# RLinf/RLinf

Measured on NVIDIA H100. Metric: env-steps/sec (rollout+update), higher is better.
Workload: dtype f32

## Files before the change

rlinf_b200/csrc/mlp.cu:

```cuda
#include <curand_kernel.h>

#include "common.cuh"
#include "sgemm.cuh"
#include "tc_gemm.cuh"

namespace {

using namespace rb::gemm;

__global__ void __launch_bounds__(256) colsum_kernel(const float* __restrict__ Z, float* __restrict__ out, int64_t M, int N,
                                                     int64_t rows_per_block) {
  const int64_t r0 = (int64_t)blockIdx.x * rows_per_block;
  const int64_t r1 = (r0 + rows_per_block < M) ? r0 + rows_per_block : M;
  for (int n = threadIdx.x; n < N; n += blockDim.x) {
    float s0 = 0.f, s1 = 0.f, s2 = 0.f, s3 = 0.f;
    int64_t r = r0;
    for (; r + 3 < r1; r += 4) {
      s0 += Z[r * N + n];
      s1 += Z[(r + 1) * N + n];
      s2 += Z[(r + 2) * N + n];
      s3 += Z[(r + 3) * N + n];
    }
    for (; r < r1; ++r) s0 += Z[r * N + n];
    atomicAdd(&out[n], (s0 + s1) + (s2 + s3));
// ... 309 lines not shown
    }
    if (lane == 0) {
      if (mz > 0.f) atomicMax(reinterpret_cast<unsigned int*>(p.amax_dz3), __float_as_uint(mz));
      if (has_v && my > 0.f && p.amax_dy3) atomicMax(reinterpret_cast<unsigned int*>(p.amax_dy3), __float_as_uint(my));
    }
  }
#pragma unroll
  for (int j = 0; j < 4; ++j) {
    atomicAdd(&a_b2[lane * 4 + j], cb[j]);
    atomicAdd(&a_b2[128 + lane * 4 + j], cb[4 + j]);
    if (has_v) {
      atomicAdd(&a_vb2[lane * 4 + j], cv[j]);
      atomicAdd(&a_vb2[128 + lane * 4 + j], cv[4 + j]);
    }
  }
  if (REG) {
#pragma unroll
    for (int a = 0; a < 8; ++a) {
      if (a >= p.act) break;
      float* am = a_mw + a * kH;
#pragma unroll
      for (int j = 0; j < 4; ++j) {
        atomicAdd(&am[lane * 4 + j], rm[a][j]);
        atomicAdd(&am[128 + lane * 4 + j], rm[a][4 + j]);
      }
    }
    if (has_v) {
#pragma unroll
      for (int c = 0; c < 2; ++c) {
        if (c >= p.vdim) break;
        float* av = a_vw + c * kH;
#pragma unroll
        for (int j = 0; j < 4; ++j) {
          atomicAdd(&av[lane * 4 + j], rv[c][j]);
          atomicAdd(&av[128 + lane * 4 + j], rv[c][4 + j]);
        }
      }
    }
  }
  __syncthreads();
  for (int i = threadIdx.x; i < acc_len; i += blockDim.x) {
    float s = 0.f;
    for (int w = 0; w < nwarp; ++w) s += acc0[w * acc_len + i];
    p.part[(size_t)blockIdx.x * acc_len + i] = s;
  }
}

int head_grid(int64_t n) {
  int64_t blocks = (n + 7) / 8;
  const int64_t cap = (int64_t)rb::sm_count() * 4;
  if (blocks > cap) blocks = cap;
  return (int)(blocks < 1 ? 1 : blocks);
}

struct TowerW {
  const float *w0, *b0, *w1, *b1, *w2, *b2;
};
int layer_forward(const float* in, const int64_t* idx, int64_t n, int in_dim, const float* w, const float* b,
                  float* out, cudaStream_t st) {
  GemmArgs g{};
  g.M = n; g.N = kH; g.ldc = kH; g.k_per_split = 1 << 30;
  g.A = in; g.lda = in_dim; g.a_rows = idx; g.B = w; g.ldb = in_dim; g.K = in_dim; g.bias = b; g.C = out;
  return launch_gemm<A_KCONTIG, B_KCONTIG, EPI_BIAS_TANH>(g, 1, st);
}

int tower_forward(const float* X, const int64_t* idx, int64_t n, int in_dim, const TowerW& w, float* H1, float* H2,
                  float* H3, cudaStream_t st) {
  int e = layer_forward(X, idx, n, in_dim, w.w0, w.b0, H1, st);
  if (e) return e;
  e = layer_forward(H1, nullptr, n, kH, w.w1, w.b1, H2, st);
  if (e) return e;
  return layer_forward(H2, nullptr, n, kH, w.w2, w.b2, H3, st);
}

int tower_backward(const float* X, const int64_t* idx, int64_t n, int in_dim, const TowerW& w, const float* H1, const float* H2, const float* dZ3, float* tmpA, float* tmpB, float* g_w0,
                   float* g_b0, float* g_w1, float* g_b1, float* g_w2, float* g_b2, cudaStream_t st) {
  const int64_t rows_per_split = 4096;
  const int splits = (int)((n + rows_per_split - 1) / rows_per_split);
  const int64_t cs_rows = 128;
  const int cs_blocks = (int)((n + cs_rows - 1) / cs_rows);
  int e;
  auto colsum = [&](const float* dZ, float* gb) -> int {
    colsum_kernel<<<cs_blocks, 256, 0, st>>>(dZ, gb, n, kH, cs_rows);
    rb::count_launch();
    cudaError_t ce = cudaPeekAtLastError();
    return ce == cudaSuccess ? 0 : (int)ce;
  };
  auto wgrad = [&](const float* dZ, const float* Hin, const int64_t* in_rows, int in_ld, float* gw, float* gb,
                   bool need_colsum) -> int {
    GemmArgs g{};
    g.A = dZ; g.lda = kH; g.B = Hin; g.ldb = in_ld; g.b_rows = in_rows; g.C = gw;
    g.ldc = in_ld; g.M = kH; g.N = in_ld; g.K = n; g.k_per_split = rows_per_split;
    const int ee = launch_gemm<A_MCONTIG, B_NCONTIG, EPI_ATOMIC>(g, splits, st);
    if (ee || !need_colsum) return ee;
    return colsum(dZ, gb);
  };
  auto dgrad = [&](const float* dZ, const float* W, const float* Hprev, float* out) -> int {
    GemmArgs g{};
    g.A = dZ; g.lda = kH; g.B = W; g.ldb = kH; g.C = out; g.ldc = kH; g.aux = Hprev;
    g.ldaux = kH; g.M = n; g.N = kH; g.K = kH; g.k_per_split = 1 << 30;
    return launch_gemm<A_KCONTIG, B_NCONTIG, EPI_TANHGRAD>(g, 1, st);
  };
  if ((e = wgrad(dZ3, H2, nullptr, kH, g_w2, g_b2, false))) return e;
  if ((e = dgrad(dZ3, w.w2, H2, tmpA))) return e;
  if ((e = wgrad(tmpA, H1, nullptr, kH, g_w1, g_b1, true))) return e;
  if ((e = dgrad(tmpA, w.w1, H1, tmpB))) return e;
  return wgrad(tmpB, X, idx, in_dim, g_w0, g_b0, true);
}


struct TowerWH {
  const float *w0f, *w1f, *w2f;
  const float *w1d, *w2d;
};

struct TowerIO {
  TowerW w;
  TowerWH wh;
  float *H1, *H2, *H3;
  float *g_w0, *g_b0, *g_w1, *g_b1, *g_w2, *g_b2;
  const float* dZ3;
  float *tA, *tB;
  float* amax;
};

bool layer0_on_tc(const int64_t* idx, int in_dim) { return idx == nullptr && in_dim % rb::tc::BK == 0; }

float* x_amax_slot(const rb200_mlp_layout* L, float* buf, int64_t n) { return buf + 6 * n * kH + n * L->act_dim; }
int64_t x_amax_floats(int cols) { return cols <= 256 ? 4 + cols : 1; }

int publish_absmax(const float* X, int64_t rows, int cols, float* out, cudaStream_t st) {
  if (reinterpret_cast<uintptr_t>(X) & 15) return RB200_E_ALIGN;
  if (cols % 4 != 0) return RB200_E_SHAPE;
  cudaError_t ce = cudaMemsetAsync(out, 0, sizeof(float) * x_amax_floats(cols), st);
  if (ce != cudaSuccess) return (int)ce;
  const int cols4 = cols / 4, col_out = cols <= 256 ? cols : 0;
  const int threads = col_out ? cols4 * (256 / cols4) : 256;
  const int64_t n4 = rows * cols4;
  int64_t blocks = (n4 + threads - 1) / threads;
  const int64_t cap = (int64_t)rb::sm_count() * 4;
  if (blocks > cap) blocks = cap;
  absmax_kernel<<<(int)(blocks < 1 ? 1 : blocks), threads, 0, st>>>(reinterpret_cast<const float4*>(X), n4,
                                                                    col_out ? cols4 : 1, col_out, out);
  rb::count_launch();
  ce = cudaPeekAtLastError();
  return ce == cudaSuccess ? 0 : (int)ce;
}

int towers_forward_h(const float* X, const int64_t* idx, int64_t n, int in_dim, TowerIO* t, int nt, float* x_amax,
                     const float* x_amax_in, cudaStream_t st) {
  int e;
  const bool l0_tc = layer0_on_tc(idx, in_dim);
  rb::tch::GemmLaunch g[2];
  if (l0_tc) {
    if (x_amax_in) {
      cudaError_t ce = cudaMemcpyAsync(x_amax, x_amax_in, sizeof(float) * x_amax_floats(in_dim), cudaMemcpyDeviceToDevice, st);
      if (ce != cudaSuccess) return (int)ce;
    } else if ((e = publish_absmax(X, n, in_dim, x_amax, st))) {
      return e;
    }
    for (int i = 0; i < nt; ++i) g[i] = rb::tch::GemmLaunch{X, t[i].wh.w0f, nullptr, t[i].H1, t[i].w.b0, nullptr, nullptr, nullptr, nullptr, x_amax};
    if ((e = rb::tch::launch(g, nt, n, in_dim, rb::tc::EPI_BIAS_TANH, 0, st))) return e;
  } else {
    for (int i = 0; i < nt; ++i)
      if ((e = layer_forward(X, idx, n, in_dim, t[i].w.w0, t[i].w.b0, t[i].H1, st))) return e;
  }
  for (int i = 0; i < nt; ++i) g[i] = rb::tch::GemmLaunch{t[i].H1, t[i].wh.w1f, nullptr, t[i].H2, t[i].w.b1, nullptr, nullptr, nullptr, nullptr};
  if ((e = rb::tch::launch(g, nt, n, kH, rb::tc::EPI_BIAS_TANH, 0, st))) return e;
  for (int i = 0; i < nt; ++i) g[i] = rb::tch::GemmLaunch{t[i].H2, t[i].wh.w2f, nullptr, t[i].H3, t[i].w.b2, nullptr, nullptr, nullptr, nullptr};
  return rb::tch::launch(g, nt, n, kH, rb::tc::EPI_BIAS_TANH, 0, st);
}

int simt_wgrad_chunks(int64_t n, int64_t* rows_per_chunk) {
  int64_t chunks = (n + 255) / 256;
  const int64_t cap = rb::sm_count() / 2 > 1 ? rb::sm_count() / 2 : 1;
  if (chunks > cap) chunks = cap;
  const int64_t rows = (n + chunks - 1) / chunks;
  *rows_per_chunk = rows;
  return (int)((n + rows - 1) / rows);
}

int towers_backward_h(const float* X, const int64_t* idx, int64_t n, int in_dim, TowerIO* t, int nt,
                      const float* x_amax, cudaStream_t st) {
  int e;
  rb::tch::WgradLaunch w[2];
  rb::tch::BackwardLaunch b[2];
  for (int i = 0; i < nt; ++i)
    b[i] = rb::tch::BackwardLaunch{t[i].dZ3, t[i].wh.w2d, t[i].H2, t[i].tA, t[i].g_w2, t[i].g_b1, t[i].amax, t[i].amax + 1,
                                   t[i].tB};
  if ((e = rb::tch::dgrad_wgrad(b, nt, n, st))) return e;
  for (int i = 0; i < nt; ++i)
    b[i] = rb::tch::BackwardLaunch{t[i].tA, t[i].wh.w1d, t[i].H1, t[i].tB, t[i].g_w1, t[i].g_b0, t[i].amax + 1, t[i].amax + 2,
                                   const_cast<float*>(t[i].dZ3)};
  if ((e = rb::tch::dgrad_wgrad(b, nt, n, st))) return e;
  if (layer0_on_tc(idx, in_dim) && in_dim <= 256) {
    for (int i = 0; i < nt; ++i) w[i] = rb::tch::WgradLaunch{t[i].tB, X, t[i].g_w0, t[i].amax + 2, x_amax + 4};
    return rb::tch::wgrad(w, nt, n, in_dim, st);
  }
  int64_t rows = 0;
  const int chunks = simt_wgrad_chunks(n, &rows);
  const int64_t slab = (int64_t)kH * in_dim;
  float* part = rb::partials_scratch(chunks * slab);
  if (!part) return RB200_E_UNSUPPORTED;
  for (int i = 0; i < nt; ++i) {
    GemmArgs a{};
    a.A = t[i].tB; a.lda = kH; a.B = X; a.ldb = in_dim; a.b_rows = idx; a.C = part; a.c_split_stride = slab;
    a.ldc = in_dim; a.M = kH; a.N = in_dim; a.K = n; a.k_per_split = rows;
    if ((e = launch_gemm<A_MCONTIG, B_NCONTIG, EPI_STORE>(a, chunks, st))) return e;
    rb::tch::SlotSums ss{};
    ss.count = 1;
    ss.nslab = chunks;
    ss.stride = slab;
    ss.part[0] = part;
    ss.out[0] = t[i].g_w0;
    ss.len[0] = (int)slab;
    if ((e = rb::tch::sum_slots(ss, st))) return e;
  }
  return 0;
}

}

extern "C" int rb200_mlp_layout_init(rb200_mlp_layout* L, int obs_dim, int act_dim, int value_dim, int hidden) {
  if (!L) return RB200_E_NULL;
  if (obs_dim <= 0 || act_dim <= 0 || value_dim < 0) return RB200_E_SHAPE;
  if (hidden != kH || act_dim > kMaxAct || value_dim > kMaxVal) return RB200_E_UNSUPPORTED;
  L->obs_dim = obs_dim; L->act_dim = act_dim; L->value_dim = value_dim; L->hidden = hidden;
  int64_t o = 0;
  auto take = [&](int64_t n) { o = (o + 3) & ~int64_t(3); const int64_t at = o; o += n; return at; };
  L->logstd = take(act_dim);
  L->vw0 = take((int64_t)hidden * obs_dim); L->vb0 = take(hidden);
  L->vw1 = take((int64_t)hidden * hidden); L->vb1 = take(hidden);
  L->vw2 = take((int64_t)hidden * hidden); L->vb2 = take(hidden);
  L->vw3 = take((int64_t)value_dim * hidden);
  L->bw0 = take((int64_t)hidden * obs_dim); L->bb0 = take(hidden);
  L->bw1 = take((int64_t)hidden * hidden); L->bb1 = take(hidden);
  L->bw2 = take((int64_t)hidden * hidden); L->bb2 = take(hidden);
  L->mw = take((int64_t)act_dim * hidden); L->mb = take(act_dim);
  L->total = (o + 3) & ~int64_t(3);
  const int64_t sms = rb::sm_count(), head = 4 * sms * ((act_dim + value_dim) * hidden + 64 + 2 * hidden);
  const int64_t wg = sms / 2 * hidden * (obs_dim > hidden ? obs_dim : hidden) + sms * hidden;
  if (!rb::partials_scratch(head > wg ? head : wg)) (void)cudaGetLastError();
  return RB200_OK;
}

static inline int64_t act_floats(int64_t n) { return n * kH; }

extern "C" int64_t rb200_mlp_fwd_scratch_floats(const rb200_mlp_layout* L, int64_t n) {
  if (!L || n <= 0) return 0;
  return 6 * act_floats(n) + n * L->act_dim + 64 + 256;
}

static inline int64_t wsplit_tower_floats(int obs) { return (int64_t)kH * obs + 4ll * kH * kH; }

extern "C" int64_t rb200_mlp_wsplit_floats(const rb200_mlp_layout* L) {
  if (!L) return 0;
  return 2 * wsplit_tower_floats(L->obs_dim);
}

static int check_layout(const rb200_mlp_layout* L) {
  if (!L) return RB200_E_NULL;
  if (L->hidden != kH || L->act_dim <= 0 || L->act_dim > kMaxAct || L->value_dim < 0 || L->value_dim > kMaxVal)
    return RB200_E_UNSUPPORTED;
  return RB200_OK;
}

namespace {
TowerW tower_w(const rb200_mlp_layout* L, const float* P, bool value) {
  TowerW w;
  if (value) {
    w.w0 = P + L->vw0; w.b0 = P + L->vb0; w.w1 = P + L->vw1; w.b1 = P + L->vb1; w.w2 = P + L->vw2; w.b2 = P + L->vb2;
  } else {
    w.w0 = P + L->bw0; w.b0 = P + L->bb0; w.w1 = P + L->bw1; w.b1 = P + L->bb1; w.w2 = P + L->bw2; w.b2 = P + L->bb2;
  }
  return w;
}
TowerWH tower_wh(const rb200_mlp_layout* L, const float* ws, bool value) {
  const int64_t n0 = (int64_t)kH * L->obs_dim, nn = (int64_t)kH * kH;
  const float* b = ws + (value ? 0 : wsplit_tower_floats(L->obs_dim));
  TowerWH t;
  t.w0f = b;
  t.w1f = b + n0;
  t.w2f = b + n0 + nn;
  t.w1d = b + n0 + 2 * nn;
  t.w2d = b + n0 + 3 * nn;
  return t;
}
}

extern "C" int rb200_mlp_prepare_weights(const rb200_mlp_layout* L, const float* params, float* wsplit,
                                         rb200_stream_t stream) {
  int e = check_layout(L);
  if (e) return e;
  if (!params || !wsplit) return RB200_E_NULL;
  rb::tch::SplitSpec sp[6];
  int cnt = 0;
  for (int v = 0; v < 2; ++v) {
    if (v == 0 && L->value_dim == 0) continue;
    const TowerW w = tower_w(L, params, v == 0);
    const TowerWH t = tower_wh(L, wsplit, v == 0);
    const int64_t n0 = (int64_t)kH * L->obs_dim, nn = (int64_t)kH * kH;
    if (L->obs_dim % rb::tc::BK == 0)
      sp[cnt++] = rb::tch::SplitSpec{w.w0, const_cast<float*>(t.w0f), nullptr, n0};
    sp[cnt++] = rb::tch::SplitSpec{w.w1, const_cast<float*>(t.w1f), const_cast<float*>(t.w1d), nn};
    sp[cnt++] = rb::tch::SplitSpec{w.w2, const_cast<float*>(t.w2f), const_cast<float*>(t.w2d), nn};
  }
  return rb::tch::split_weights(sp, cnt, rb::as_stream(stream));
}

extern "C" int rb200_mlp_forward(const rb200_mlp_layout* L, const float* params, const float* wsplit,
                                 const float* states, const float* action, const int64_t* idx, int64_t n,
                                 float* logprobs, float* entropy, float* values, float* acts, float* work,
                                 const float* states_amax, rb200_stream_t stream) {
  int e = check_layout(L);
  if (e) return e;
  if (!params || !states || !action || !logprobs || !acts || !work) return RB200_E_NULL;
  if (n <= 0) return RB200_E_SHAPE;
  if (values && L->value_dim == 0) return RB200_E_SHAPE;
  cudaStream_t st = rb::as_stream(stream);
  const int64_t PF = act_floats(n);
  float *H1 = acts, *H2 = H1 + PF, *H3 = H2 + PF, *G1 = H3 + PF, *G2 = G1 + PF, *G3 = G2 + PF;
  float* mean = G3 + PF;
  const float* P = params;
// ... 219 lines not shown
```

rlinf_b200/csrc/tc_gemm.cuh:

```cuda
#pragma once
#include <cuda_runtime.h>
#include <stdint.h>

namespace rb {
namespace tc {

constexpr int BM = 128, BN = 256, BK = 32;

enum Epi { EPI_STORE = 0, EPI_BIAS_TANH = 1, EPI_TANHGRAD = 2 };

extern int g_debug_flags;

}

namespace tch {

struct GemmLaunch {
  const float* a;
  const float* b_hi;
  const float* b_lo;
  float* c;
  const float* bias;
  const float* h;
  float* colsum;
  const float* amax_in;
  float* amax_out;
  const float* amax_x;
};
struct WgradLaunch {
  const float* z;
  const float* h;
  float* dW;
  const float* amax_z;
  const float* amax_h;
};
struct SplitSpec {
  const float* src;
  float* hi;
  float* lo;
  int64_t n;
};

int launch(const GemmLaunch* groups, int ngroups, int64_t M, int K, int epi, int b_mn, cudaStream_t st);
int wgrad(const WgradLaunch* groups, int ngroups, int64_t n, int IN, cudaStream_t st);
struct BackwardLaunch {
  const float* z;
  const float* wpack;
  const float* h;
  float* dzprev;
  float* dW;
  float* colsum;
  const float* amax_in;
  float* amax_out;
  float* scratch;
};
int dgrad_wgrad(const BackwardLaunch* groups, int ngroups, int64_t n, cudaStream_t st);
int split_weights(const SplitSpec* specs, int count, cudaStream_t st);
struct SlotSums {
  const float* part[8];
  float* out[8];
  int len[8];
  int count, nslab;
  int64_t stride;
};
int sum_slots(const SlotSums& s, cudaStream_t st);

}
}
```

rlinf_b200/csrc/tc_gemm_h.cu:

```cuda
#include <cuda_fp16.h>

#include "common.cuh"
#include "tc_gemm.cuh"
#include "tc_half.cuh"
#include "tma.cuh"
#include "wgmma.cuh"

namespace rb {
namespace tch {

using rb::tc::BK;
using rb::tc::BM;
using rb::tc::BN;

constexpr int kStages = 4;
constexpr int kA32 = BM * BK * 4;
constexpr int kB16 = BN * BK * 2;
constexpr int kWBytes = 2 * kB16;
constexpr int kStageBytes = kA32 + kWBytes;
constexpr int kRingBytes = kStages * kStageBytes;
constexpr int kThreads = 384;
constexpr int kProducerRegs = 40, kConsumerRegs = 232;
static_assert(128 * kProducerRegs + 256 * kConsumerRegs <= 65536, "register file");

__device__ __forceinline__ float tanh_fast(float x) {
  const float t = __expf(-2.0f * fabsf(x));
  return copysignf(__fdividef(1.0f - t, 1.0f + t), x);
}

__device__ __forceinline__ void a_frag_rows(const uint8_t* tile, int r0, int c0, float scale, uint32_t (&hi)[4],
                                            uint32_t (&lo)[4]) {
#pragma unroll
  for (int i = 0; i < 4; ++i) {
    const int r = r0 + (i & 1) * 8, c = c0 + (i >> 1) * 8;
    const float2 x = *reinterpret_cast<const float2*>(tile + r * 128 + ((((c >> 2) ^ (r & 7))) << 4) + (c & 3) * 4);
    split2(x.x * scale, x.y * scale, hi[i], lo[i]);
  }
}

struct __align__(16) Barriers {
  uint64_t full[kStages];
  uint64_t empty[kStages];
  alignas(16) float bias[BN];
  float csum[8][BN];
};

struct Group {
  const float* bias;
  const float* h;
  float* colsum;
  const float* amax_in;
  const float* amax_x;
  float* amax_out;
  float* c;
};

struct GemmParams {
  CUtensorMap a[2];
  const uint8_t* wpack[2];
  Group g[2];
  float* part;
  int64_t M;
  int K;
  int epi;
  int ngroups;
};

template <int B_MN>
__global__ void __launch_bounds__(kThreads, 1) tc_h_gemm_kernel(const __grid_constant__ GemmParams P) {
  extern __shared__ uint8_t smem_raw[];
  uint8_t* smem = smem_raw + ((1024u - (tma::smem_u32(smem_raw) & 1023u)) & 1023u);
  Barriers* bars = reinterpret_cast<Barriers*>(smem + kRingBytes);

  const int wg = threadIdx.x >> 7, warp = threadIdx.x >> 5, lane = threadIdx.x & 31;
  const int grp = blockIdx.x % P.ngroups;
  const int cta = blockIdx.x / P.ngroups, n_cta = gridDim.x / P.ngroups;
  const Group& G = P.g[grp];
  const int64_t n_tiles = (P.M + BM - 1) / BM;
  const int n_kb = P.K / BK;

  if (threadIdx.x == 0) {
    for (int s = 0; s < kStages; ++s) {
      tma::mbar_init(&bars->full[s], 1);
      tma::mbar_init(&bars->empty[s], 8);
    }
    tma::fence_barrier_init();
  }
  for (int i = threadIdx.x; i < BN; i += kThreads) bars->bias[i] = (P.epi == rb::tc::EPI_BIAS_TANH) ? G.bias[i] : 0.f;
  for (int i = threadIdx.x; i < 8 * BN; i += kThreads) bars->csum[i / BN][i % BN] = 0.f;
  __syncthreads();

  if (wg == 2) {
    wg::setmaxnreg_dec<kProducerRegs>();
    if (threadIdx.x == 256) {
      tma::prefetch_desc(&P.a[grp]);
      uint32_t s = 0, ph = 0;
      for (int64_t tile = cta; tile < n_tiles; tile += n_cta) {
        for (int kb = 0; kb < n_kb; ++kb) {
          tma::mbar_wait(&bars->empty[s], ph ^ 1u);
          uint8_t* st = smem + s * kStageBytes;
          tma::mbar_arrive_expect_tx(&bars->full[s], kStageBytes);
          tma::load_2d(st, &P.a[grp], kb * BK, (int)(tile * BM), &bars->full[s]);
          bulk_load(st + kA32, P.wpack[grp] + (size_t)kb * kWBytes, kWBytes, &bars->full[s]);
          if (++s == kStages) { s = 0; ph ^= 1u; }
        }
      }
    }
  } else {
    wg::setmaxnreg_inc<kConsumerRegs>();
    const int cw = wg;
    const int g = lane >> 2, t = lane & 3;
    const int r_lo = cw * 64 + (warp & 3) * 16 + g;
    const int sa = G.amax_in ? scale_log2_for(__ldg(G.amax_in)) : (G.amax_x ? input_scale_log2_for(__ldg(G.amax_x)) : 0);
    const float a_scale = pow2i(sa);
    const float out_scale = pow2i(-(sa + kWeightScaleLog2));
    float vmax = 0.f;
    auto load_a = [&](uint32_t q, uint32_t(&ah)[BK / 16][4], uint32_t(&al)[BK / 16][4]) {
      tma::mbar_wait_brk(&bars->full[q % kStages], (q / kStages) & 1u);
      const uint8_t* st = smem + (q % kStages) * kStageBytes;
#pragma unroll
      for (int k = 0; k < BK / 16; ++k) a_frag_rows(st, r_lo, k * 16 + 2 * t, a_scale, ah[k], al[k]);
    };
    uint32_t q0 = 0;
    for (int64_t tile = cta; tile < n_tiles; tile += n_cta) {
      float acc[128];
#pragma unroll
      for (int i = 0; i < 128; ++i) acc[i] = 0.f;
      auto step = [&](int kb, const uint32_t(&ah)[BK / 16][4], const uint32_t(&al)[BK / 16][4],
                      uint32_t(&nh)[BK / 16][4], uint32_t(&nl)[BK / 16][4]) {
        const uint32_t q = q0 + kb;
        const uint32_t wbase = tma::smem_u32(smem + (q % kStages) * kStageBytes + kA32);
        wg::fence();
#pragma unroll
        for (int k = 0; k < BK / 16; ++k) {
          const uint64_t b_hi = B_MN ? wg::desc(wbase + k * 2048, 4096, 1024, kSw128) : wg::desc(wbase + k * 32, 16, 512, kSw64);
          const uint64_t b_lo = B_MN ? wg::desc(wbase + kB16 + k * 2048, 4096, 1024, kSw128)
                                     : wg::desc(wbase + kB16 + k * 32, 16, 512, kSw64);
          wg::Mma<256, B_MN>::run(acc, al[k], b_hi, 1u);
          wg::Mma<256, B_MN>::run(acc, ah[k], b_lo, 1u);
          wg::Mma<256, B_MN>::run(acc, ah[k], b_hi, 1u);
        }
        wg::commit();
        wg::wait<1>();
        if (kb > 0) warp_arrive(&bars->empty[(q - 1) % kStages]);
        if (kb + 1 < n_kb) load_a(q + 1, nh, nl);
      };
      uint32_t ah0[BK / 16][4], al0[BK / 16][4], ah1[BK / 16][4], al1[BK / 16][4];
      load_a(q0, ah0, al0);
      for (int kb = 0; kb < n_kb; kb += 2) {
        step(kb, ah0, al0, ah1, al1);
        if (kb + 1 < n_kb) step(kb + 1, ah1, al1, ah0, al0);
      }
      wg::wait<0>();
      q0 += n_kb;
      warp_arrive(&bars->empty[(q0 - 1) % kStages]);
      const int64_t row0 = tile * BM + r_lo, row1 = row0 + 8;
      const bool ok0 = row0 < P.M, ok1 = row1 < P.M;
#pragma unroll
      for (int j = 0; j < BN / 8; ++j) {
        const int col = 8 * j + 2 * t;
        float v0 = acc[4 * j] * out_scale, v1 = acc[4 * j + 1] * out_scale;
        float v2 = acc[4 * j + 2] * out_scale, v3 = acc[4 * j + 3] * out_scale;
        if (P.epi == rb::tc::EPI_BIAS_TANH) {
          const float2 b = *reinterpret_cast<const float2*>(&bars->bias[col]);
          v0 = tanh_fast(v0 + b.x); v1 = tanh_fast(v1 + b.y);
          v2 = tanh_fast(v2 + b.x); v3 = tanh_fast(v3 + b.y);
        } else if (P.epi == rb::tc::EPI_TANHGRAD) {
          const float2 h0 = ok0 ? __ldg(reinterpret_cast<const float2*>(G.h + row0 * BN + col)) : make_float2(0.f, 0.f);
          const float2 h1 = ok1 ? __ldg(reinterpret_cast<const float2*>(G.h + row1 * BN + col)) : make_float2(0.f, 0.f);
          v0 = ok0 ? v0 * (1.0f - h0.x * h0.x) : 0.f; v1 = ok0 ? v1 * (1.0f - h0.y * h0.y) : 0.f;
          v2 = ok1 ? v2 * (1.0f - h1.x * h1.x) : 0.f; v3 = ok1 ? v3 * (1.0f - h1.y * h1.y) : 0.f;
          vmax = fmaxf(vmax, fmaxf(fmaxf(fabsf(v0), fabsf(v1)), fmaxf(fabsf(v2), fabsf(v3))));
          if (G.colsum != nullptr) {
            float c0 = v0 + v2, c1 = v1 + v3;
#pragma unroll
            for (int o = 4; o < 32; o <<= 1) {
              c0 += __shfl_xor_sync(0xffffffffu, c0, o);
              c1 += __shfl_xor_sync(0xffffffffu, c1, o);
            }
            if (g == 0) {
              bars->csum[warp][col] += c0;
              bars->csum[warp][col + 1] += c1;
            }
          }
        }
        if (ok0) *reinterpret_cast<float2*>(G.c + row0 * BN + col) = make_float2(v0, v1);
        if (ok1) *reinterpret_cast<float2*>(G.c + row1 * BN + col) = make_float2(v2, v3);
      }
    }
    if (G.amax_out != nullptr && P.epi == rb::tc::EPI_TANHGRAD) {
#pragma unroll
// ... 242 lines not shown

int launch(const GemmLaunch* L, int ngroups, int64_t M, int K, int epi, int b_mn, cudaStream_t st) {
  if (ngroups < 1 || ngroups > 2 || K % BK != 0 || K <= 0 || M <= 0) return RB200_E_SHAPE;
  GemmParams P{};
  P.M = M; P.K = K; P.epi = epi; P.ngroups = ngroups;
  for (int g = 0; g < ngroups; ++g) {
    const GemmLaunch& l = L[g];
    const uintptr_t al = reinterpret_cast<uintptr_t>(l.a) | reinterpret_cast<uintptr_t>(l.b_hi) |
                         reinterpret_cast<uintptr_t>(l.c) | reinterpret_cast<uintptr_t>(l.h);
    if (al & 15) return RB200_E_ALIGN;
    if (encode_f32_sw128(&P.a[g], l.a, (uint64_t)M, (uint64_t)K, BM)) return RB200_E_UNSUPPORTED;
    P.wpack[g] = reinterpret_cast<const uint8_t*>(l.b_hi);
    P.g[g] = Group{l.bias, l.h, l.colsum, l.amax_in, l.amax_x, l.amax_out, l.c};
  }
  static bool attr_done = false;
  constexpr int kSmem = kRingBytes + 1024 + (int)sizeof(Barriers);
  static_assert(kSmem <= 232448, "tc_h_gemm_kernel shared memory");
  if (!attr_done) {
    cudaError_t ce = cudaFuncSetAttribute(tc_h_gemm_kernel<0>, cudaFuncAttributeMaxDynamicSharedMemorySize, kSmem);
    if (ce == cudaSuccess) ce = cudaFuncSetAttribute(tc_h_gemm_kernel<1>, cudaFuncAttributeMaxDynamicSharedMemorySize, kSmem);
    if (ce != cudaSuccess) return (int)ce;
    attr_done = true;
  }
  const int64_t n_tiles = (M + BM - 1) / BM;
  int per_group = rb::sm_count() / ngroups;
  if (per_group > n_tiles) per_group = (int)n_tiles;
  if (per_group < 1) per_group = 1;
  rb::tch::SlotSums ss{};
  ss.nslab = per_group;
  ss.stride = (int64_t)ngroups * BN;
  if (epi == rb::tc::EPI_TANHGRAD)
    for (int g = 0; g < ngroups; ++g)
      if (L[g].colsum) {
        if (!P.part && !(P.part = rb::partials_scratch((int64_t)per_group * ngroups * BN))) return RB200_E_UNSUPPORTED;
        ss.part[ss.count] = P.part + g * BN;
        ss.out[ss.count] = L[g].colsum;
        ss.len[ss.count++] = BN;
      }
  if (b_mn) tc_h_gemm_kernel<1><<<per_group * ngroups, kThreads, kSmem, st>>>(P);
  else tc_h_gemm_kernel<0><<<per_group * ngroups, kThreads, kSmem, st>>>(P);
  rb::count_launch();
  cudaError_t ce = cudaPeekAtLastError();
  if (ce != cudaSuccess) return (int)ce;
  return ss.count ? rb::tch::sum_slots(ss, st) : 0;
}

int wgrad(const WgradLaunch* L, int ngroups, int64_t n, int IN, cudaStream_t st) {
  if (ngroups < 1 || ngroups > 2 || n <= 0 || IN <= 0 || IN > 256 || IN % 32 != 0) return RB200_E_SHAPE;
  WgradParams P{};
  P.n = n; P.IN = IN; P.ngroups = ngroups;
  for (int g = 0; g < ngroups; ++g) {
    const uintptr_t al = reinterpret_cast<uintptr_t>(L[g].z) | reinterpret_cast<uintptr_t>(L[g].h) |
                         reinterpret_cast<uintptr_t>(L[g].dW);
    if (al & 15) return RB200_E_ALIGN;
    int e = encode_f32_sw128(&P.z[g], L[g].z, (uint64_t)n, 256, 32);
    if (!e) e = encode_f32_sw128(&P.h[g], L[g].h, (uint64_t)n, (uint64_t)IN, 32);
    if (e) return RB200_E_UNSUPPORTED;
    P.dW[g] = L[g].dW;
    P.amax_z[g] = L[g].amax_z;
    P.amax_h[g] = L[g].amax_h;
  }
  static bool attr_done = false;
  constexpr int kSmem = kWgRingBytes + 1024 + (int)sizeof(WgBarriers);
  static_assert(kSmem <= 232448, "tc_h_wgrad_kernel shared memory");
  if (!attr_done) {
    cudaError_t ce = cudaFuncSetAttribute(tc_h_wgrad_kernel<128>, cudaFuncAttributeMaxDynamicSharedMemorySize, kSmem);
    if (ce == cudaSuccess) ce = cudaFuncSetAttribute(tc_h_wgrad_kernel<256>, cudaFuncAttributeMaxDynamicSharedMemorySize, kSmem);
    if (ce != cudaSuccess) return (int)ce;
    attr_done = true;
  }
  const int n_kb = (int)((n + BK - 1) / BK);
  int chunks = rb::sm_count() / (2 * ngroups);
  if (chunks < 1) chunks = 1;
  if (chunks > n_kb) chunks = n_kb;
  P.kb_per_chunk = (n_kb + chunks - 1) / chunks;
  chunks = (n_kb + P.kb_per_chunk - 1) / P.kb_per_chunk;
  const int64_t slab = 256 * (int64_t)IN;
  if (!(P.part = rb::partials_scratch(chunks * ngroups * slab))) return RB200_E_UNSUPPORTED;
  const dim3 grid(ngroups * 2 * chunks);
  if (IN <= 128) tc_h_wgrad_kernel<128><<<grid, kThreads, kSmem, st>>>(P);
  else tc_h_wgrad_kernel<256><<<grid, kThreads, kSmem, st>>>(P);
  rb::count_launch();
  cudaError_t ce = cudaPeekAtLastError();
  if (ce != cudaSuccess) return (int)ce;
  rb::tch::SlotSums ss{};
  ss.count = ngroups;
  ss.nslab = chunks;
  ss.stride = ngroups * slab;
  for (int g = 0; g < ngroups; ++g) {
    ss.part[g] = P.part + g * slab;
    ss.out[g] = L[g].dW;
    ss.len[g] = (int)slab;
  }
  return rb::tch::sum_slots(ss, st);
}

__global__ void __launch_bounds__(256) sum_slots_kernel(const SlotSums s) {
  const int q = blockIdx.y;
  for (int i = blockIdx.x * blockDim.x + threadIdx.x; i < s.len[q]; i += gridDim.x * blockDim.x) {
    float acc = 0.f;
    for (int k = 0; k < s.nslab; ++k) acc += s.part[q][k * s.stride + i];
    s.out[q][i] += acc;
  }
}

int sum_slots(const SlotSums& s, cudaStream_t st) {
  if (s.count < 1 || s.count > 8 || s.nslab < 1) return RB200_E_SHAPE;
  int len = 0;
  for (int q = 0; q < s.count; ++q) len = s.len[q] > len ? s.len[q] : len;
  int blocks = (len + 255) / 256;
  if (blocks > 4 * rb::sm_count()) blocks = 4 * rb::sm_count();
  sum_slots_kernel<<<dim3(blocks, s.count), 256, 0, st>>>(s);
  rb::count_launch();
  cudaError_t ce = cudaPeekAtLastError();
  return ce == cudaSuccess ? 0 : (int)ce;
}

int split_weights(const SplitSpec* specs, int count, cudaStream_t st) {
  if (count < 1 || count > 8) return RB200_E_SHAPE;
  SplitJobs jobs{};
  jobs.count = count;
  int64_t total = 0;
  for (int i = 0; i < count; ++i) {
    const int64_t K = specs[i].n / BN;
    if (K * BN != specs[i].n || K % BK != 0 || (specs[i].lo != nullptr && K != BN)) return RB200_E_SHAPE;
    jobs.j[i] = SplitJob{specs[i].src, reinterpret_cast<uint8_t*>(specs[i].hi), reinterpret_cast<uint8_t*>(specs[i].lo), (int)K};
    total = specs[i].n / 8 > total ? specs[i].n / 8 : total;
  }
  int64_t blocks = (total + 255) / 256;
  const int64_t cap = (int64_t)rb::sm_count() * 4;
  if (blocks > cap) blocks = cap;
  split_half_kernel<<<(int)blocks, 256, 0, st>>>(jobs);
  rb::count_launch();
  cudaError_t ce = cudaPeekAtLastError();
  return ce == cudaSuccess ? 0 : (int)ce;
}

}

namespace tc {
int g_debug_flags = 0;

}
}

extern "C" int rb200_debug_set_flags(int flags) {
  rb::tc::g_debug_flags = flags;
  return RB200_OK;
}

extern "C" int rb200_tc_gemm_h(const float* A, const float* B, float* C, int64_t M, int K, int mode, const float* amax,
                               float* work, rb200_stream_t stream) {
  if (!A || !B || !C || !work) return RB200_E_NULL;
  if (M <= 0 || K <= 0 || K % rb::tc::BK != 0) return RB200_E_SHAPE;
  cudaStream_t st = rb::as_stream(stream);
  const int64_t nb = (int64_t)rb::tc::BN * K;
  if (mode && K != rb::tc::BN) return RB200_E_SHAPE;
  rb::tch::SplitSpec sp{B, work, mode ? work + nb : nullptr, nb};
  int e = rb::tch::split_weights(&sp, 1, st);
  if (e) return e;
  rb::tch::GemmLaunch l{};
  l.a = A; l.b_hi = mode ? sp.lo : sp.hi; l.b_lo = nullptr; l.c = C; l.amax_in = amax;
  return rb::tch::launch(&l, 1, M, K, rb::tc::EPI_STORE, mode ? 1 : 0, st);
}

extern "C" int rb200_tc_wgrad_h(const float* Z, const float* H, float* dW, int64_t n, int IN, const float* amax,
                                rb200_stream_t stream) {
  if (!Z || !H || !dW) return RB200_E_NULL;
  rb::tch::WgradLaunch l{Z, H, dW, amax};
  return rb::tch::wgrad(&l, 1, n, IN, rb::as_stream(stream));
}
```

rlinf_b200/csrc/tc_half.cuh:

```cuda
#pragma once
#include <cuda_fp16.h>
#include <stdint.h>

#include "tma.cuh"

namespace rb {
namespace tch {

constexpr int kWeightScaleLog2 = 10;

__device__ __forceinline__ void bulk_load(void* smem_dst, const void* gsrc, uint32_t bytes, uint64_t* bar) {
  asm volatile("cp.async.bulk.shared::cluster.global.mbarrier::complete_tx::bytes [%0], [%1], %2, [%3];" ::"r"(
                   tma::smem_u32(smem_dst)),
               "l"(reinterpret_cast<uint64_t>(gsrc)), "r"(bytes), "r"(tma::smem_u32(bar))
               : "memory");
}
__device__ __forceinline__ void warp_arrive(uint64_t* bar) {
  __syncwarp();
  if ((threadIdx.x & 31) == 0) tma::mbar_arrive(bar);
}

constexpr uint32_t kSw128 = 1, kSw64 = 2;

__device__ __forceinline__ float pow2i(int s) { return __int_as_float((s + 127) << 23); }
__device__ __forceinline__ int scale_log2_for(float amax) {
  const int e = (int)((__float_as_uint(amax) >> 23) & 0xffu) - 127;
  if (!(amax > 0.0f) || e < -120) return 0;
  int s = 13 - e;
  return s > 100 ? 100 : (s < -100 ? -100 : s);
}

__device__ __forceinline__ int input_scale_log2_for(float amax) {
  const int e = (int)((__float_as_uint(amax) >> 23) & 0xffu) - 127;
  return (e >= -1 && e <= 14) ? 0 : scale_log2_for(amax);
}

__device__ __forceinline__ void split2(float x0, float x1, uint32_t& hi, uint32_t& lo) {
  const __half2 hh = __floats2half2_rn(x0, x1);
  const float2 hf = __half22float2(hh);
  const __half2 ll = __floats2half2_rn(x0 - hf.x, x1 - hf.y);
  hi = *reinterpret_cast<const uint32_t*>(&hh);
  lo = *reinterpret_cast<const uint32_t*>(&ll);
}

__device__ __forceinline__ void split_item(const uint8_t* src, int r, int cp, float scale, uint4& hi, uint4& lo) {
  const uint8_t* srow = src + r * 128;
  const float4 x0 = *reinterpret_cast<const float4*>(srow + (((2 * cp) ^ (r & 7)) << 4));
  const float4 x1 = *reinterpret_cast<const float4*>(srow + (((2 * cp + 1) ^ (r & 7)) << 4));
  split2(x0.x * scale, x0.y * scale, hi.x, lo.x);
  split2(x0.z * scale, x0.w * scale, hi.y, lo.y);
  split2(x1.x * scale, x1.y * scale, hi.z, lo.z);
  split2(x1.z * scale, x1.w * scale, hi.w, lo.w);
}
__device__ __forceinline__ void split_item_cols(const uint8_t* src, int r, int cp, const float* sc, uint4& hi, uint4& lo) {
  const uint8_t* srow = src + r * 128;
  const float4 x0 = *reinterpret_cast<const float4*>(srow + (((2 * cp) ^ (r & 7)) << 4));
  const float4 x1 = *reinterpret_cast<const float4*>(srow + (((2 * cp + 1) ^ (r & 7)) << 4));
  const float4 s0 = *reinterpret_cast<const float4*>(sc), s1 = *reinterpret_cast<const float4*>(sc + 4);
  split2(x0.x * s0.x, x0.y * s0.y, hi.x, lo.x);
  split2(x0.z * s0.z, x0.w * s0.w, hi.y, lo.y);
  split2(x1.x * s1.x, x1.y * s1.y, hi.z, lo.z);
  split2(x1.z * s1.z, x1.w * s1.w, hi.w, lo.w);
}
__device__ __forceinline__ int split_item_dst(int r, int cp) { return r * 64 + ((cp ^ ((r >> 1) & 3)) << 4); }

template <int NT>
__device__ __forceinline__ void split_tile(const uint8_t* __restrict__ src, uint8_t* __restrict__ hi, uint8_t* __restrict__ lo,
                                           int rows, int t, float scale) {
  const int items = rows * 4;
#pragma unroll 2
  for (int i = t; i < items; i += NT) {
    const int r = i >> 2, cp = i & 3;
    uint4 h, l;
    split_item(src, r, cp, scale, h, l);
    *reinterpret_cast<uint4*>(hi + split_item_dst(r, cp)) = h;
    *reinterpret_cast<uint4*>(lo + split_item_dst(r, cp)) = l;
  }
}

__device__ __forceinline__ void split_box_in_place(uint8_t* box, int lane, float scale) {
  uint4 h[4], l[4];
#pragma unroll
  for (int j = 0; j < 4; ++j) split_item(box, (lane >> 2) + 8 * j, lane & 3, scale, h[j], l[j]);
  __syncwarp();
#pragma unroll
  for (int j = 0; j < 4; ++j) {
    const int d = split_item_dst((lane >> 2) + 8 * j, lane & 3);
    *reinterpret_cast<uint4*>(box + d) = h[j];
    *reinterpret_cast<uint4*>(box + 2048 + d) = l[j];
  }
}

}
}
```

Before: 6.400 million.

## Add weight-stationary forward GEMM kernel for K at most BN

Adds a dedicated forward tensor-core kernel for the tower MLP layers with K up to BN. Each CTA keeps its half of the split-fp16 weights resident in shared memory, loaded once by TMA. It then streams 64-row activation tiles through per-consumer rings across three consumer warpgroups, with register fragments double-buffered. The aim is to avoid reloading weights per tile and to improve overlap compared with the generic 128x256 launch path. The cost is a new, more complex kernel with its own register and shared-memory budget, plus more code paths to keep correct.

```diff
diff --git a/rlinf_b200/csrc/mlp.cu b/rlinf_b200/csrc/mlp.cu
--- a/rlinf_b200/csrc/mlp.cu
+++ b/rlinf_b200/csrc/mlp.cu
@@ -485,6 +485,10 @@
   int e;
   const bool l0_tc = layer0_on_tc(idx, in_dim);
   rb::tch::GemmLaunch g[2];
+  auto gemm = [&](int K) {
+    return K <= rb::tc::BN ? rb::tch::forward(g, nt, n, K, rb::tc::EPI_BIAS_TANH, st)
+                           : rb::tch::launch(g, nt, n, K, rb::tc::EPI_BIAS_TANH, 0, st);
+  };
   if (l0_tc) {
     if (x_amax_in) {
       cudaError_t ce = cudaMemcpyAsync(x_amax, x_amax_in, sizeof(float) * x_amax_floats(in_dim), cudaMemcpyDeviceToDevice, st);
@@ -493,15 +497,15 @@
       return e;
     }
     for (int i = 0; i < nt; ++i) g[i] = rb::tch::GemmLaunch{X, t[i].wh.w0f, nullptr, t[i].H1, t[i].w.b0, nullptr, nullptr, nullptr, nullptr, x_amax};
-    if ((e = rb::tch::launch(g, nt, n, in_dim, rb::tc::EPI_BIAS_TANH, 0, st))) return e;
+    if ((e = gemm(in_dim))) return e;
   } else {
     for (int i = 0; i < nt; ++i)
       if ((e = layer_forward(X, idx, n, in_dim, t[i].w.w0, t[i].w.b0, t[i].H1, st))) return e;
   }
   for (int i = 0; i < nt; ++i) g[i] = rb::tch::GemmLaunch{t[i].H1, t[i].wh.w1f, nullptr, t[i].H2, t[i].w.b1, nullptr, nullptr, nullptr, nullptr};
-  if ((e = rb::tch::launch(g, nt, n, kH, rb::tc::EPI_BIAS_TANH, 0, st))) return e;
+  if ((e = gemm(kH))) return e;
   for (int i = 0; i < nt; ++i) g[i] = rb::tch::GemmLaunch{t[i].H2, t[i].wh.w2f, nullptr, t[i].H3, t[i].w.b2, nullptr, nullptr, nullptr, nullptr};
-  return rb::tch::launch(g, nt, n, kH, rb::tc::EPI_BIAS_TANH, 0, st);
+  return gemm(kH);
 }
 
 int simt_wgrad_chunks(int64_t n, int64_t* rows_per_chunk) {
diff --git a/rlinf_b200/csrc/tc_forward_h.cu b/rlinf_b200/csrc/tc_forward_h.cu
--- /dev/null
+++ b/rlinf_b200/csrc/tc_forward_h.cu
@@ -0,0 +1,207 @@
+#include <cuda_fp16.h>
+
+#include "common.cuh"
+#include "tc_gemm.cuh"
+#include "tc_half.cuh"
+#include "tma.cuh"
+#include "wgmma.cuh"
+
+namespace rb {
+namespace tch {
+
+using rb::tc::BK;
+using rb::tc::BN;
+
+constexpr int kFwdRows = 64;
+constexpr int kFwdCols = BN / 2;
+constexpr int kFwdBox = kFwdRows * BK * 4;
+constexpr int kFwdW16 = kFwdCols * BK * 2;
+constexpr int kFwdWkb = 2 * kFwdW16;
+constexpr int kFwdWAll = (BN / BK) * kFwdWkb;
+constexpr int kFwdConsumers = 3;
+constexpr int kFwdStages = 4;
+constexpr int kFwdRingBytes = kFwdConsumers * kFwdStages * kFwdBox;
+constexpr int kFwdThreads = 128 * (kFwdConsumers + 1);
+constexpr int kFwdLaunchRegs = 65536 / kFwdThreads / 8 * 8;
+constexpr int kFwdProducerRegs = 40, kFwdConsumerRegs = 152;
+static_assert(128 * (kFwdLaunchRegs - kFwdProducerRegs) >= 128 * kFwdConsumers * (kFwdConsumerRegs - kFwdLaunchRegs),
+              "register pool");
+
+struct FwdBarriers {
+  uint64_t full[kFwdConsumers][kFwdStages];
+  uint64_t empty[kFwdConsumers][kFwdStages];
+  uint64_t w_full;
+  alignas(16) float bias[kFwdCols];
+};
+
+struct FwdGroup {
+  const float* bias;
+  const float* amax_in;
+  const float* amax_x;
+  float* c;
+};
+
+struct FwdParams {
+  CUtensorMap a[2];
+  const uint8_t* wpack[2];
+  FwdGroup g[2];
+  int64_t M;
+  int K, ngroups;
+};
+
+__global__ void __launch_bounds__(kFwdThreads, 1) tc_h_fwd_kernel(const __grid_constant__ FwdParams P) {
+  extern __shared__ uint8_t smem_raw[];
+  uint8_t* smem = smem_raw + ((1024u - (tma::smem_u32(smem_raw) & 1023u)) & 1023u);
+  uint8_t* wst = smem + kFwdRingBytes;
+  FwdBarriers* bars = reinterpret_cast<FwdBarriers*>(wst + kFwdWAll);
+  const int wg = threadIdx.x >> 7, warp = threadIdx.x >> 5, lane = threadIdx.x & 31;
+  const int half = blockIdx.x & 1, grp = (blockIdx.x >> 1) % P.ngroups;
+  const int cta = blockIdx.x / (2 * P.ngroups), n_cta = gridDim.x / (2 * P.ngroups);
+  const FwdGroup& G = P.g[grp];
+  const int64_t n_tiles = (P.M + kFwdRows - 1) / kFwdRows;
+  const int n_kb = P.K / BK;
+
+  if (threadIdx.x == 0) {
+    for (int w = 0; w < kFwdConsumers; ++w)
+      for (int s = 0; s < kFwdStages; ++s) {
+        tma::mbar_init(&bars->full[w][s], 1);
+        tma::mbar_init(&bars->empty[w][s], 4);
+      }
+    tma::mbar_init(&bars->w_full, 1);
+    tma::fence_barrier_init();
+  }
+  for (int i = threadIdx.x; i < kFwdCols; i += kFwdThreads) bars->bias[i] = G.bias ? G.bias[half * kFwdCols + i] : 0.f;
+  __syncthreads();
+
+  if (wg == kFwdConsumers) {
+    wg::setmaxnreg_dec<kFwdProducerRegs>();
+    const int w = warp - 4 * kFwdConsumers;
+    if (lane == 0 && w < kFwdConsumers) {
+      tma::prefetch_desc(&P.a[grp]);
+      if (w == 0) {
+        const uint8_t* wsrc = P.wpack[grp] + half * kFwdW16;
+        tma::mbar_arrive_expect_tx(&bars->w_full, n_kb * kFwdWkb);
+        for (int kb = 0; kb < n_kb; ++kb) {
+          bulk_load(wst + kb * kFwdWkb, wsrc + (size_t)kb * 4 * kFwdW16, kFwdW16, &bars->w_full);
+          bulk_load(wst + kb * kFwdWkb + kFwdW16, wsrc + (size_t)kb * 4 * kFwdW16 + 2 * kFwdW16, kFwdW16, &bars->w_full);
+        }
+      }
+      uint8_t* ring = smem + w * kFwdStages * kFwdBox;
+      uint32_t s = 0, ph = 0;
+      for (int64_t tile = cta + (int64_t)w * n_cta; tile < n_tiles; tile += (int64_t)kFwdConsumers * n_cta) {
+        for (int kb = 0; kb < n_kb; ++kb) {
+          tma::mbar_wait(&bars->empty[w][s], ph ^ 1u);
+          tma::mbar_arrive_expect_tx(&bars->full[w][s], kFwdBox);
+          tma::load_2d(ring + s * kFwdBox, &P.a[grp], kb * BK, (int)(tile * kFwdRows), &bars->full[w][s]);
+          if (++s == kFwdStages) { s = 0; ph ^= 1u; }
+        }
+      }
+    }
+  } else {
+    wg::setmaxnreg_inc<kFwdConsumerRegs>();
+    const int g = lane >> 2, t = lane & 3;
+    const int r_lo = (warp & 3) * 16 + g;
+    const int sa = G.amax_in ? scale_log2_for(__ldg(G.amax_in)) : (G.amax_x ? input_scale_log2_for(__ldg(G.amax_x)) : 0);
+    const float a_scale = pow2i(sa);
+    const float out_scale = pow2i(-(sa + kWeightScaleLog2));
+    const bool tanh_out = G.bias != nullptr;
+    float* cbase = G.c + half * kFwdCols;
+    const uint32_t w0 = tma::smem_u32(wst);
+    const uint8_t* ring = smem + wg * kFwdStages * kFwdBox;
+    uint64_t* full = bars->full[wg];
+    uint64_t* empty = bars->empty[wg];
+    auto load_a = [&](uint32_t q, uint32_t(&ah)[BK / 16][4], uint32_t(&al)[BK / 16][4]) {
+      tma::mbar_wait_brk(&full[q % kFwdStages], (q / kFwdStages) & 1u);
+      const uint8_t* st = ring + (q % kFwdStages) * kFwdBox;
+#pragma unroll
+      for (int k = 0; k < BK / 16; ++k) a_frag_rows(st, r_lo, k * 16 + 2 * t, a_scale, ah[k], al[k]);
+    };
+    tma::mbar_wait_brk(&bars->w_full, 0u);
+    for (int64_t j = wg;; j += kFwdConsumers) {
+      const int64_t tile = cta + j * n_cta;
+      if (tile >= n_tiles) break;
+      const uint32_t q0 = (uint32_t)(j / kFwdConsumers) * n_kb;
+      float acc[64];
+#pragma unroll
+      for (int i = 0; i < 64; ++i) acc[i] = 0.f;
+      auto step = [&](int kb, const uint32_t(&ah)[BK / 16][4], const uint32_t(&al)[BK / 16][4],
+                      uint32_t(&nh)[BK / 16][4], uint32_t(&nl)[BK / 16][4]) {
+        const uint32_t wb = w0 + kb * kFwdWkb;
+        wg::fence();
+#pragma unroll
+        for (int k = 0; k < BK / 16; ++k) {
+          const uint64_t b_hi = wg::desc(wb + k * 32, 16, 512, kSw64);
+          const uint64_t b_lo = wg::desc(wb + kFwdW16 + k * 32, 16, 512, kSw64);
+          wg::Mma<128, 0>::run(acc, al[k], b_hi, 1u);
+          wg::Mma<128, 0>::run(acc, ah[k], b_lo, 1u);
+          wg::Mma<128, 0>::run(acc, ah[k], b_hi, 1u);
+        }
+        wg::commit();
+        warp_arrive(&empty[(q0 + kb) % kFwdStages]);
+        wg::wait<1>();
+        if (kb + 1 < n_kb) load_a(q0 + kb + 1, nh, nl);
+      };
+      uint32_t ah0[BK / 16][4], al0[BK / 16][4], ah1[BK / 16][4], al1[BK / 16][4];
+      load_a(q0, ah0, al0);
+      for (int kb = 0; kb < n_kb; kb += 2) {
+        step(kb, ah0, al0, ah1, al1);
+        if (kb + 1 < n_kb) step(kb + 1, ah1, al1, ah0, al0);
+      }
+      wg::wait<0>();
+      wg::fence_operand(acc);
+      const int64_t row0 = tile * kFwdRows + r_lo, row1 = row0 + 8;
+      const bool ok0 = row0 < P.M, ok1 = row1 < P.M;
+#pragma unroll
+      for (int jj = 0; jj < kFwdCols / 8; ++jj) {
+        const int col = 8 * jj + 2 * t;
+        float v0 = acc[4 * jj] * out_scale, v1 = acc[4 * jj + 1] * out_scale;
+        float v2 = acc[4 * jj + 2] * out_scale, v3 = acc[4 * jj + 3] * out_scale;
+        if (tanh_out) {
+          const float2 b = *reinterpret_cast<const float2*>(&bars->bias[col]);
+          v0 = tanh_fast(v0 + b.x); v1 = tanh_fast(v1 + b.y);
+          v2 = tanh_fast(v2 + b.x); v3 = tanh_fast(v3 + b.y);
+        }
+        if (ok0) *reinterpret_cast<float2*>(cbase + row0 * BN + col) = make_float2(v0, v1);
+        if (ok1) *reinterpret_cast<float2*>(cbase + row1 * BN + col) = make_float2(v2, v3);
+      }
+    }
+  }
+}
+
+int encode_f32_sw128(CUtensorMap* out, const float* base, uint64_t rows, uint64_t cols, uint32_t box_rows);
+
+int forward(const GemmLaunch* L, int ngroups, int64_t M, int K, int epi, cudaStream_t st) {
+  if (ngroups < 1 || ngroups > 2 || K % BK != 0 || K <= 0 || K > BN || M <= 0) return RB200_E_SHAPE;
+  if (epi != rb::tc::EPI_STORE && epi != rb::tc::EPI_BIAS_TANH) return RB200_E_UNSUPPORTED;
+  FwdParams P{};
+  P.M = M; P.K = K; P.ngroups = ngroups;
+  for (int g = 0; g < ngroups; ++g) {
+    const GemmLaunch& l = L[g];
+    const uintptr_t al = reinterpret_cast<uintptr_t>(l.a) | reinterpret_cast<uintptr_t>(l.b_hi) |
+                         reinterpret_cast<uintptr_t>(l.c);
+    if (al & 15) return RB200_E_ALIGN;
+    if (epi == rb::tc::EPI_BIAS_TANH && !l.bias) return RB200_E_NULL;
+    if (encode_f32_sw128(&P.a[g], l.a, (uint64_t)M, (uint64_t)K, kFwdRows)) return RB200_E_UNSUPPORTED;
+    P.wpack[g] = reinterpret_cast<const uint8_t*>(l.b_hi);
+    P.g[g] = FwdGroup{epi == rb::tc::EPI_BIAS_TANH ? l.bias : nullptr, l.amax_in, l.amax_x, l.c};
+  }
+  static bool attr_done = false;
+  constexpr int kSmem = kFwdRingBytes + kFwdWAll + 1024 + (int)sizeof(FwdBarriers);
+  static_assert(kSmem <= 232448, "tc_h_fwd_kernel shared memory");
+  if (!attr_done) {
+    const cudaError_t ce = cudaFuncSetAttribute(tc_h_fwd_kernel, cudaFuncAttributeMaxDynamicSharedMemorySize, kSmem);
+    if (ce != cudaSuccess) return (int)ce;
+    attr_done = true;
+  }
+  const int64_t n_tiles = (M + kFwdRows - 1) / kFwdRows;
+  int n_cta = rb::sm_count() / (2 * ngroups);
+  if (n_cta > n_tiles) n_cta = (int)n_tiles;
+  if (n_cta < 1) n_cta = 1;
+  tc_h_fwd_kernel<<<n_cta * ngroups * 2, kFwdThreads, kSmem, st>>>(P);
+  rb::count_launch();
+  const cudaError_t ce = cudaPeekAtLastError();
+  return ce == cudaSuccess ? 0 : (int)ce;
+}
+
+}
+}
diff --git a/rlinf_b200/csrc/tc_gemm.cuh b/rlinf_b200/csrc/tc_gemm.cuh
--- a/rlinf_b200/csrc/tc_gemm.cuh
+++ b/rlinf_b200/csrc/tc_gemm.cuh
@@ -42,6 +42,7 @@
 };
 
 int launch(const GemmLaunch* groups, int ngroups, int64_t M, int K, int epi, int b_mn, cudaStream_t st);
+int forward(const GemmLaunch* groups, int ngroups, int64_t M, int K, int epi, cudaStream_t st);
 int wgrad(const WgradLaunch* groups, int ngroups, int64_t n, int IN, cudaStream_t st);
 struct BackwardLaunch {
   const float* z;
diff --git a/rlinf_b200/csrc/tc_gemm_h.cu b/rlinf_b200/csrc/tc_gemm_h.cu
--- a/rlinf_b200/csrc/tc_gemm_h.cu
+++ b/rlinf_b200/csrc/tc_gemm_h.cu
@@ -22,21 +22,6 @@
 constexpr int kThreads = 384;
 constexpr int kProducerRegs = 40, kConsumerRegs = 232;
 static_assert(128 * kProducerRegs + 256 * kConsumerRegs <= 65536, "register file");
-
-__device__ __forceinline__ float tanh_fast(float x) {
-  const float t = __expf(-2.0f * fabsf(x));
-  return copysignf(__fdividef(1.0f - t, 1.0f + t), x);
-}
-
-__device__ __forceinline__ void a_frag_rows(const uint8_t* tile, int r0, int c0, float scale, uint32_t (&hi)[4],
-                                            uint32_t (&lo)[4]) {
-#pragma unroll
-  for (int i = 0; i < 4; ++i) {
-    const int r = r0 + (i & 1) * 8, c = c0 + (i >> 1) * 8;
-    const float2 x = *reinterpret_cast<const float2*>(tile + r * 128 + ((((c >> 2) ^ (r & 7))) << 4) + (c & 3) * 4);
-    split2(x.x * scale, x.y * scale, hi[i], lo[i]);
-  }
-}
 
 struct __align__(16) Barriers {
   uint64_t full[kStages];
@@ -585,16 +570,18 @@
 extern "C" int rb200_tc_gemm_h(const float* A, const float* B, float* C, int64_t M, int K, int mode, const float* amax,
                                float* work, rb200_stream_t stream) {
   if (!A || !B || !C || !work) return RB200_E_NULL;
-  if (M <= 0 || K <= 0 || K % rb::tc::BK != 0) return RB200_E_SHAPE;
+  if (M <= 0 || K <= 0 || K % rb::tc::BK != 0 || mode < 0 || mode > 2) return RB200_E_SHAPE;
   cudaStream_t st = rb::as_stream(stream);
   const int64_t nb = (int64_t)rb::tc::BN * K;
-  if (mode && K != rb::tc::BN) return RB200_E_SHAPE;
-  rb::tch::SplitSpec sp{B, work, mode ? work + nb : nullptr, nb};
+  const bool dgrad = mode == 1;
+  if (dgrad && K != rb::tc::BN) return RB200_E_SHAPE;
+  rb::tch::SplitSpec sp{B, work, dgrad ? work + nb : nullptr, nb};
   int e = rb::tch::split_weights(&sp, 1, st);
   if (e) return e;
   rb::tch::GemmLaunch l{};
-  l.a = A; l.b_hi = mode ? sp.lo : sp.hi; l.b_lo = nullptr; l.c = C; l.amax_in = amax;
-  return rb::tch::launch(&l, 1, M, K, rb::tc::EPI_STORE, mode ? 1 : 0, st);
+  l.a = A; l.b_hi = dgrad ? sp.lo : sp.hi; l.b_lo = nullptr; l.c = C; l.amax_in = amax;
+  if (mode == 0 && K <= rb::tc::BN) return rb::tch::forward(&l, 1, M, K, rb::tc::EPI_STORE, st);
+  return rb::tch::launch(&l, 1, M, K, rb::tc::EPI_STORE, dgrad ? 1 : 0, st);
 }
 
 extern "C" int rb200_tc_wgrad_h(const float* Z, const float* H, float* dW, int64_t n, int IN, const float* amax,
diff --git a/rlinf_b200/csrc/tc_half.cuh b/rlinf_b200/csrc/tc_half.cuh
--- a/rlinf_b200/csrc/tc_half.cuh
+++ b/rlinf_b200/csrc/tc_half.cuh
@@ -41,6 +41,21 @@
   const __half2 ll = __floats2half2_rn(x0 - hf.x, x1 - hf.y);
   hi = *reinterpret_cast<const uint32_t*>(&hh);
   lo = *reinterpret_cast<const uint32_t*>(&ll);
+}
+
+__device__ __forceinline__ void a_frag_rows(const uint8_t* tile, int r0, int c0, float scale, uint32_t (&hi)[4],
+                                            uint32_t (&lo)[4]) {
+#pragma unroll
+  for (int i = 0; i < 4; ++i) {
+    const int r = r0 + (i & 1) * 8, c = c0 + (i >> 1) * 8;
+    const float2 x = *reinterpret_cast<const float2*>(tile + r * 128 + ((((c >> 2) ^ (r & 7))) << 4) + (c & 3) * 4);
+    split2(x.x * scale, x.y * scale, hi[i], lo[i]);
+  }
+}
+
+__device__ __forceinline__ float tanh_fast(float x) {
+  const float t = __expf(-2.0f * fabsf(x));
+  return copysignf(__fdividef(1.0f - t, 1.0f + t), x);
 }
 
 __device__ __forceinline__ void split_item(const uint8_t* src, int r, int cp, float scale, uint4& hi, uint4& lo) {
```

Result: faster. 6.615 million, median of 6 (+3.4%).
